# open-mmlab/Amphion

Hardware: AMD Instinct MI355X
Metric: audio samples/sec (HiFi-GAN V1 22.05 kHz generator, mel->wav) (higher is better)
Workload: dtype f32 (split-f16 MFMA: 3 x v_mfma_f32_32x32x16_f16 per term, f32 accumulate)

## Files before the change

### amphion_amd/_lib.py

```python
from __future__ import annotations

import ctypes
import os
import weakref
from ctypes import POINTER, c_char_p, c_float, c_int, c_int32, c_int64, c_size_t, c_void_p

_HERE = os.path.dirname(os.path.abspath(__file__))
LIB_PATH = os.environ.get("AMP_LIB_PATH") or os.path.join(_HERE, "lib", "libamphion_hip.so")

AMP_MAX_STAGES = 8
AMP_MAX_KERNELS = 8
AMP_MAX_DILATIONS = 8

AMP_ARCH_HIFIGAN, AMP_ARCH_BIGVGAN, AMP_ARCH_HIFIGAN_VITS = 0, 1, 2
AMP_ACT_LRELU, AMP_ACT_SNAKE, AMP_ACT_SNAKEBETA = 0, 1, 2
AMP_PRECISION_F32, AMP_PRECISION_F16X3 = 0, 1
AMP_CONV_OPT_PAD_REFLECT, AMP_CONV_OPT_TANH = 1, 2
AMP_PAD_REPLICATE, AMP_PAD_ZEROS, AMP_PAD_REFLECT = 0, 1, 2
AMP_PW_BIAS, AMP_PW_BIAS_GELU, AMP_PW_SCALE_RES = 0, 1, 2
PRECISIONS = {"f32": AMP_PRECISION_F32, "fp32": AMP_PRECISION_F32, "f16x3": AMP_PRECISION_F16X3}


class AmpError(RuntimeError):

# ... 161 lines not shown
    "amp_dsconv_forward": (c_int, [c_void_p, c_void_p, c_int, c_int, c_int, c_void_p, c_size_t, c_void_p, c_void_p]),
    "amp_dsconv_destroy": (None, [c_void_p]),
    "amp_gelu": (c_int, [c_void_p, ctypes.c_longlong, c_void_p, c_void_p]),
    "amp_layer_norm_c": (c_int, [c_void_p, c_void_p, c_void_p, c_void_p, c_void_p, c_int, c_int, c_int, c_float, c_int, c_void_p, c_void_p]),
    "amp_add_channel_bias": (c_int, [c_void_p, c_void_p, c_int, c_int, c_int, c_void_p]),
    "amp_layer_norm_c_ragged": (c_int, [c_void_p, c_void_p, c_void_p, c_void_p, c_void_p, c_void_p, c_int, c_int, c_int, c_float, c_int, c_void_p, c_void_p]),
    "amp_dds_seam": (c_int, [c_void_p, c_void_p, c_void_p, c_void_p, c_float, c_void_p, c_void_p, c_int, c_int, c_void_p, c_void_p, c_float,
                             c_void_p, c_int, c_int, c_int, c_void_p, c_void_p, c_void_p]),
    "amp_dwconv_layer_norm_c": (c_int, [c_void_p, c_void_p, c_void_p, c_int, c_int, c_void_p, c_void_p, c_void_p, c_int, c_int, c_int, c_float, c_int, c_void_p, c_void_p]),
    "amp_dwconv_layer_norm_c_causal": (c_int, [c_void_p, c_void_p, c_void_p, c_int, c_int, c_void_p, c_void_p, c_void_p, c_int, c_int, c_int, c_float, c_int,
                                               c_void_p, c_void_p]),
    "amp_rel_attention_strided": (c_int, [c_void_p, c_void_p, c_void_p, ctypes.c_longlong, c_void_p, c_void_p, c_void_p, c_int, c_int, c_int, c_int, c_int, c_void_p, c_void_p]),
    "amp_set_rel_attention_tiled": (c_int, [c_int]),
    "amp_set_resblock_streams": (c_int, [c_int]),
    "amp_gen_prepare_streams": (c_int, [c_void_p]),
    "amp_rel_attention": (c_int, [c_void_p, c_void_p, c_void_p, c_void_p, c_void_p, c_void_p, c_int, c_int, c_int, c_int, c_int, c_void_p, c_void_p]),
    "amp_dwconv": (c_int, [c_void_p, c_void_p, c_void_p, c_void_p, c_int, c_int, c_int, c_int, c_int, c_void_p, c_void_p]),
    "amp_spline_flow": (c_int, [c_void_p, c_void_p, c_void_p, c_int, c_int, c_int, c_int, c_float, c_int, c_int, c_int, c_void_p, c_void_p]),
    "amp_spline_flow_proj": (c_int, [c_void_p, c_void_p, c_void_p, c_void_p, c_void_p, c_int, c_int, c_int, c_int, c_int, c_float, c_int, c_int, c_int, c_void_p, c_void_p]),
    "amp_affine_reverse": (c_int, [c_void_p, c_void_p, c_void_p, c_void_p, c_int, c_int, c_int, c_void_p, c_void_p]),
    "amp_embed_tokens": (c_int, [c_void_p, c_void_p, c_void_p, c_int, c_int, c_int, c_int, c_float, c_void_p, c_void_p]),
    "amp_durations": (c_int, [c_void_p, c_void_p, c_int, c_int, c_float, c_void_p, c_void_p, c_void_p, c_void_p]),
    "amp_expand_path": (c_int, [c_void_p, c_void_p, c_void_p, c_void_p, c_int, c_int, c_int, c_int, c_void_p, c_void_p, c_void_p]),
    "amp_expand_path_strided": (c_int, [c_void_p, ctypes.c_longlong, c_void_p, c_void_p, c_void_p, c_int, c_int, c_int, c_int, c_void_p, c_void_p, c_void_p]),
    "amp_gauss_sample": (c_int, [c_void_p, c_void_p, c_void_p, c_size_t, c_float, c_void_p, c_void_p]),
    "amp_snake": (c_int, [c_void_p, c_int, c_int, c_int, c_void_p, c_void_p, c_int, c_void_p, c_void_p]),
    "amp_fir_upsample": (c_int, [c_void_p, c_int, c_int, c_int, c_void_p, c_int, c_int, c_void_p, c_void_p]),
    "amp_fir_filter": (c_int, [c_void_p, c_int, c_int, c_int, c_void_p, c_int, c_int, c_int, c_int, c_int, c_void_p, c_void_p]),
    "amp_wav_to_pcm16": (c_int, [c_void_p, c_int, c_int, ctypes.c_longlong, c_void_p, c_void_p, ctypes.c_longlong, c_void_p]),
    "amp_conv_set_option": (c_int, [c_void_p, c_int, c_int]),
    "amp_pair_forward": (c_int, [c_void_p, c_void_p, c_void_p, c_int, c_int, c_float, c_void_p, c_void_p]),
    "amp_resblock_forward": (c_int, [POINTER(c_void_p), POINTER(c_void_p), c_int, c_void_p, c_int, c_int, c_float, c_void_p, c_void_p]),
    "amp_set_resblock_fusion": (c_int, [c_int]),
    "amp_conv_destroy": (None, [c_void_p]),
    "amp_set_small_conv": (c_int, [c_int]),
    "amp_set_conv_blk": (c_int, [c_int]),
    "amp_set_conv_rg_fast": (c_int, [c_int]),
    "amp_set_pingpong": (c_int, [c_int]),
    "amp_set_conv_blk_narrow": (c_int, [c_int]),
    "amp_ampblock_forward": (c_int, [POINTER(c_void_p), POINTER(c_void_p), c_int, c_void_p, c_void_p, c_int, c_void_p, c_void_p,
                                     c_void_p, c_int, c_int, c_void_p, c_int, c_float, c_void_p]),
    "amp_set_ampblock_fusion": (c_int, [c_int]),
    "amp_conv_create_gated": (c_int, [c_int, c_int, c_int, c_int, c_void_p, c_void_p, POINTER(c_void_p)]),
    "amp_wn_forward": (c_int, [POINTER(c_void_p), POINTER(c_void_p), c_int, c_void_p, c_void_p, ctypes.c_longlong, c_void_p, c_int, c_int,
                               c_void_p, c_void_p, c_void_p]),
    "amp_wn_gate": (c_int, [c_void_p, c_void_p, ctypes.c_longlong, c_void_p, c_int, c_int, c_int, c_void_p]),
    "amp_wn_accumulate": (c_int, [c_void_p, c_void_p, c_void_p, c_void_p, c_int, c_int, c_int, c_int, c_int, c_void_p]),
    "amp_sequence_mask": (c_int, [c_void_p, c_void_p, c_int, c_int, c_int, c_void_p]),
    "amp_coupling_apply": (c_int, [c_void_p, c_void_p, c_void_p, c_int, c_int, c_int, c_int, c_void_p]),
    "amp_flip_channels": (c_int, [c_void_p, c_void_p, c_int, c_int, c_int, c_void_p]),
    "amp_posterior_sample": (c_int, [c_void_p, c_void_p, c_void_p, c_void_p, c_int, c_int, c_int, c_void_p]),
    "amp_antialias_snake": (c_int, [c_void_p, c_int, c_int, c_int, c_void_p, c_void_p, c_int, c_void_p, c_void_p, c_void_p, c_void_p]),
    "amp_istft_forward": (c_int, [POINTER(amp_mel_desc), c_void_p, c_void_p, c_int, c_int, c_void_p, c_void_p, c_void_p, c_void_p, c_void_p]),
    "amp_mel_num_frames": (c_int, [POINTER(amp_mel_desc), c_int]),
    "amp_mel_init": (c_int, []),
    "amp_mel_forward_ragged": (c_int, [POINTER(amp_mel_desc), c_void_p, c_void_p, c_int, c_int, c_void_p, c_void_p, c_void_p, c_void_p, c_void_p, c_void_p, c_void_p]),
    "amp_mel_backward": (c_int, [POINTER(amp_mel_desc), c_void_p, c_int, c_int] + [c_void_p] * 11),
    "amp_mel_forward": (c_int, [POINTER(amp_mel_desc), c_void_p, c_int, c_int, c_void_p, c_void_p, c_void_p, c_void_p, c_void_p, c_void_p, c_void_p]),
}

EXPORTED_SYMBOLS = tuple(_SIGNATURES)

_lib = None


def lib():
# ... 106 lines not shown
```

### amphion_amd/csrc/amp_host.h

```cpp
#pragma once
#include <math.h>

#include <vector>

#include "amp_internal.h"

#define AMP_HIP(expr)                                                                  \
    do {                                                                               \
        hipError_t e__ = (expr);                                                       \
        if (e__ != hipSuccess) {                                                       \
            set_error("%s failed: %s (%s:%d)", #expr, hipGetErrorString(e__), __FILE__, __LINE__); \
            return AMP_ERR_HIP;                                                        \
        }                                                                              \
    } while (0)

#define AMP_RC(expr) do { int rc__ = (expr); if (rc__ != AMP_OK) return rc__; } while (0)

struct amp_conv {
    int transposed = 0, cin = 0, cout = 0, k = 0, stride = 1, dilation = 1, padding = 0;
    int M = 0, ntaps = 0, KT = 0, off0 = 0, dstep = 0, halo_left = 0, halo_right = 0, up = 1, up_pad = 0;
    int nchunks = 0;
    int precision = amp::PREC_F32;
    int pad_reflect = 0, tanh_out = 0;
    int out_pad = 0;
// ... 93 lines not shown
    return wp;
}

template <class View>
int pack_matrix_f16x3(const char* who, int rows, int cols, int row_blocks, int k16, View W, std::vector<_Float16>* wp, float* inv_scale) {
    float wmax = 0.f;
    for (int m = 0; m < rows; ++m)
        for (int i = 0; i < cols; ++i) {
            const float w = fabsf(W(m, i));
            if (!(w < 1e30f)) { set_error("%s: non-finite weight", who); return AMP_ERR_INVALID; }
            wmax = fmaxf(wmax, w);
        }
    const float wscale = pow2_weight_scale(wmax);
    *inv_scale = 1.f / (16.f * wscale);
    *wp = pack_a_f16x3(row_blocks, k16, 1, 0, wscale, [&](int m, int i, int) { return (m < rows && i < cols) ? W(m, i) : 0.f; });
    return AMP_OK;
}

int conv_build(amp_conv* c, const float* w, const float* bias);
int conv_run(const amp_conv* c, const float* x, int B, int T, float slope_in, const float* res, float slope_out, float* y, int mode, float div,
             hipStream_t stream, long long xbs = 0, const int* lens = nullptr, int len_mul = 1, ConvArgs* plan_small = nullptr,
             int* plan_ni = nullptr);
int next_rev(const int* lens);

bool pair_supported(const amp_conv* c1, const amp_conv* c2);
int pair_run(const amp_conv* c1, const amp_conv* c2, const float* x, int B, int T, float slope, float* y, int mode, float div,
             hipStream_t stream, const int* lens = nullptr, int len_mul = 1);
bool pair_strip_plan(int B, int T, int k, bool ragged, int* form, int* strip_len, int* spi, int* steps);
bool pair_tile_args(const amp_conv* c1, const amp_conv* c2, const float* x, int B, int T, float slope, float* y, int mode, float div,
                    const int* lens, int len_mul, PairArgs* out);

bool rb_supported(const amp_conv* const* c1, const amp_conv* const* c2, int np, int B, int T);
int rb_split(const amp_conv* const* c1, int np, int B, int T);
int rb_run(const amp_conv* const* c1, const amp_conv* const* c2, int np, const float* x, int B, int T, float slope, float* y, int mode,
           float div, hipStream_t stream, const int* lens = nullptr, int len_mul = 1, int first = 0, int count = -1);

struct ActParams {
    float* a_dev = nullptr;
    float* invb_dev = nullptr;
    float* fu_dev = nullptr;
    float* fd_dev = nullptr;
    float* fu2_dev = nullptr;
};
int act_params_upload(const float* alpha_dev, const float* beta_dev, int C, int logscale, const float* filt_up_host,
                      const float* filt_down_host, float** out);
bool ampb_supported(const amp_conv* const* c1, const amp_conv* const* c2, int np, const ActParams* acts, size_t nacts, int B, int T);
int ampb_run(const amp_conv* const* c1, const amp_conv* const* c2, int np, const ActParams* acts, const float* x, int B, int T, float* y,
             int mode, float div, hipStream_t stream, const int* lens = nullptr, int len_mul = 1);

}
```

### amphion_amd/csrc/amp_internal.h

```cpp
#pragma once
#include <hip/hip_runtime.h>
#include <stdarg.h>
#include <stdint.h>
#include <stdio.h>

#include <atomic>
#include <mutex>
#include <string>
#include <vector>

#include "amphion_hip.h"

namespace amp {

constexpr int KC = 8;
constexpr int KC16 = 16;

enum { PREC_F32 = 0, PREC_F16X3 = 1 };

struct ConvArgs {
    const float* x;
    const void* wp;
    const float* bias;
    const float* res;
// ... 50 lines not shown
    float div;
    const int* lens;
    int len_mul;
    unsigned* range_flag;
};

struct ConvSmall3Args {
    ConvArgs a[3];
    int nx[3], ny[3];
};
hipError_t launch_conv_small3(const ConvSmall3Args& p, const int ni[3], hipStream_t stream);

struct Pair3Args {
    PairArgs a[3];
    int n[3];
};
hipError_t launch_pair3(const Pair3Args& p, hipStream_t stream);

constexpr int AMP_RB_MAX_PAIRS = 3;
struct RbArgs {
    const float* x;
    float* y;
    const void* wp1[AMP_RB_MAX_PAIRS];
    const float* bias1[AMP_RB_MAX_PAIRS];
    const void* wp2[AMP_RB_MAX_PAIRS];
    const float* bias2[AMP_RB_MAX_PAIRS];
    float sc1[AMP_RB_MAX_PAIRS], isc1[AMP_RB_MAX_PAIRS], sc2[AMP_RB_MAX_PAIRS], isc2[AMP_RB_MAX_PAIRS];
    int dil[AMP_RB_MAX_PAIRS];
    int np;
    int rh;
    int B, C, T;
    int tiles_per_item;
    int rev;
    float slope;
    int mode;
    float div;
    const int* lens;
    int len_mul;
    unsigned* range_flag;
};

constexpr int AMP_AMPB_MAX_STEPS = 6;
struct AmpbArgs {
    const float* x;
    float* y;
    const void* wp[AMP_AMPB_MAX_STEPS];
    const float* bias[AMP_AMPB_MAX_STEPS];
    float sc[AMP_AMPB_MAX_STEPS], isc[AMP_AMPB_MAX_STEPS];
    int dil[AMP_AMPB_MAX_STEPS];
    const float* act_a[AMP_AMPB_MAX_STEPS];
    const float* act_invb[AMP_AMPB_MAX_STEPS];
    const float* act_fu[AMP_AMPB_MAX_STEPS];
    const float* act_fd[AMP_AMPB_MAX_STEPS];
    int ns;
    int rh;
    int B, C, T;
    int tiles_per_item;
    int rev;
    int mode;
    float div;
    const int* lens;
    int len_mul;
    unsigned* range_flag;
};

constexpr int DW_TN = 64;
// ... 228 lines not shown
```

### amphion_amd/csrc/conv_host.hip

```cpp
#include <string.h>

#include <memory>
#include <type_traits>
#include <vector>

#include "amp_host.h"

namespace amp {

template <int... K> struct Taps { static constexpr int list[] = {K...}; };
using ConvTaps = Taps<1, 2, 3, 5, 7, 11>;
using BlkTaps = Taps<2, 3, 7, 11>;
using SmallTaps = Taps<1, 3, 5, 7, 11>;
using PairTaps = Taps<3, 5, 7, 11>;
using RbTaps = Taps<3, 5, 7, 11>;
using AmpbTaps = Taps<3, 5, 7, 11>;

template <int... K, typename R, typename F>
static R with_taps(Taps<K...>, int k, R dflt, F&& f) {
    R r = dflt;
    (void)((k == K && (r = f(std::integral_constant<int, K>{}), true)) || ...);
    return r;
}

// ... 396 lines not shown

bool rb_supported(const amp_conv* const* c1, const amp_conv* const* c2, int np, int B, int T) {
    if (np < 1 || np > AMP_RB_MAX_PAIRS) return false;
    int max_dil = 1, rh = 0;
    for (int p = 0; p < np; ++p) {
        if (!c1[p] || !c2[p] || !pair_supported(c1[p], c2[p])) return false;
        if (c1[p]->cin != c1[0]->cin || c1[p]->k != c1[0]->k) return false;
        max_dil = c1[p]->dilation > max_dil ? c1[p]->dilation : max_dil;
        rh += (c1[p]->k - 1) / 2 * (c1[p]->dilation + 1);
    }
    const int form = rb_form(c1[0]->cin, c1[0]->k);
    if (form < 0) return false;
    const int W = rb_tile(c1[0]->k, c1[0]->cin, max_dil, form);
    if (W <= 0 || W - 2 * rh < W / 2) return false;
    const int NT = W - 2 * rh;
    if (rb_fusion_mode() == 1 && (long long)B * ((T + NT - 1) / NT) < kRbMinWorkgroups) return false;
    return true;
}

int rb_split(const amp_conv* const* c1, int np, int B, int T) {
    if (np != 3 || rb_fusion_mode() != 1) return 0;
    int max_dil = 1, rh = 0;
    for (int p = 0; p < np; ++p) {
        max_dil = c1[p]->dilation > max_dil ? c1[p]->dilation : max_dil;
        rh += (c1[p]->k - 1) / 2 * (c1[p]->dilation + 1);
    }
    const int W = rb_tile(c1[0]->k, c1[0]->cin, max_dil, rb_form(c1[0]->cin, c1[0]->k));
    const int NT = W - 2 * rh;
    if (W <= 0 || 5 * NT >= 4 * W) return 0;
    if ((long long)B * ((T + NT - 1) / NT) < 1024) return 0;
    return 2;
}

int rb_run(const amp_conv* const* c1, const amp_conv* const* c2, int np, const float* x, int B, int T, float slope, float* y, int mode,
           float div, hipStream_t stream, const int* lens, int len_mul, int first, int count) {
    if (x == y) { set_error("rb_run: x and y must not alias"); return AMP_ERR_INVALID; }
    if (slope > 1.f) { set_error("rb_run: leaky_relu slope %g > 1 is outside the fused kernels", (double)slope); return AMP_ERR_UNSUPPORTED; }
    RbArgs a{};
    a.x = x; a.y = y;
    a.np = count < 0 ? np - first : count;
    c1 += first;
    c2 += first;
    int max_dil = 1;
    for (int p = 0; p < a.np; ++p) {
        a.wp1[p] = c1[p]->wp_dev; a.bias1[p] = c1[p]->bias_dev; a.wp2[p] = c2[p]->wp_dev; a.bias2[p] = c2[p]->bias_dev;
        a.sc1[p] = 16.f * c1[p]->wscale; a.isc1[p] = 1.f / a.sc1[p];
        a.sc2[p] = 16.f * c2[p]->wscale; a.isc2[p] = 1.f / a.sc2[p];
        a.dil[p] = c1[p]->dilation;
        a.rh += (c1[p]->k - 1) / 2 * (c1[p]->dilation + 1);
        max_dil = c1[p]->dilation > max_dil ? c1[p]->dilation : max_dil;
    }
    for (int p = a.np; p < AMP_RB_MAX_PAIRS; ++p) {
        a.wp1[p] = a.wp1[0]; a.bias1[p] = a.bias1[0]; a.wp2[p] = a.wp2[0]; a.bias2[p] = a.bias2[0]; a.dil[p] = 1;
    }
    a.B = B; a.C = c1[0]->cin; a.T = T;
    const int form = rb_form(a.C, c1[0]->k);
    const int W = rb_tile(c1[0]->k, a.C, max_dil, form);
    const int NT = W - 2 * a.rh;
    a.tiles_per_item = (T + NT - 1) / NT;
    a.slope = slope; a.mode = mode; a.div = div;
    a.lens = lens; a.len_mul = len_mul;
    a.range_flag = range_flag_for_current_device();
    a.rev = next_rev(lens);
    AMP_HIP(launch_rb(c1[0]->k, a, form, stream));
    return AMP_OK;
}

static int ampb_fusion_mode() { return cfg().ampb_fusion; }
static int ampb_form(int C, int k) {
    const int m = ampb_fusion_mode();
    if (m == 0) return -1;
    if (m == 3) return C == 32 ? 0 : 1;
    if (m == 2) return 1;
    if (C == 32) return k >= 11 ? 1 : 0;
    if (C == 64) return k <= 3 ? 1 : -1;
    return -1;
}
constexpr long long kAmpbMinWorkgroups = 256;

static int ampb_halo(const amp_conv* const* c1, int np) {
    int rh = 0;
    for (int p = 0; p < np; ++p) rh += 10 + (c1[p]->k - 1) / 2 * (c1[p]->dilation + 1);
    return (rh + 3) & ~3;
}

bool ampb_supported(const amp_conv* const* c1, const amp_conv* const* c2, int np, const ActParams* acts, size_t nacts, int B, int T) {
    if (np < 1 || 2 * np > AMP_AMPB_MAX_STEPS || nacts != (size_t)(2 * np)) return false;
    for (size_t i = 0; i < nacts; ++i)
        if (!acts[i].fu2_dev) return false;
    if ((T & 3) != 0) return false;
    int max_dil = 1;
    for (int p = 0; p < np; ++p) {
        const amp_conv *a = c1[p], *b = c2[p];
        if (!a || !b || a->precision != PREC_F16X3 || b->precision != PREC_F16X3) return false;
        if (a->pad_reflect || b->pad_reflect || a->tanh_out || b->tanh_out || a->transposed || b->transposed) return false;
        if (a->cin != a->cout || b->cin != b->cout || a->cin != b->cin || a->cin != c1[0]->cin) return false;
// ... 275 lines not shown
```

### amphion_amd/csrc/f16x3_device.h

```cpp
#pragma once
#include "amp_internal.h"

namespace amp {

typedef float f32x16 __attribute__((ext_vector_type(16)));
typedef _Float16 f16x8 __attribute__((ext_vector_type(8)));

union Frag {
    uint4 u;
    f16x8 h;
};

#define AMP_PIN_VMEM() __builtin_amdgcn_sched_barrier(0x386)
#define AMP_OPAQUE(v) asm("" : "+v"(v))

__device__ __forceinline__ int tile_order(unsigned bid, int nbx, bool ragged, int rev) {
    int bx = ((nbx & 7) == 0 && !ragged) ? (int)(bid & 7) * (nbx >> 3) + (int)(bid >> 3) : (int)bid;
    if (rev) bx = nbx - 1 - bx;
    return bx;
}

__device__ __forceinline__ int acc_row(int r, int hi = 0, int base = 0) { return base + (r & 3) + 8 * (r >> 2) + 4 * hi; }
__device__ __forceinline__ int bplane_idx(int qd, int col, int S) { return (((qd >> 1) * S + col) << 1) + (qd & 1); }
__device__ __forceinline__ void raise_range(unsigned* flag, float range_max, int lane) {
    if (flag && __any(range_max > 65504.f) && lane == 0) atomicOr(flag, 1u);
}

template <int MI, int NI>
__device__ __forceinline__ void mfma3_tiles(f32x16 (*acc)[NI], const Frag* a_h, const Frag* a_l, const Frag* bh, const Frag* bl) {
#pragma unroll
    for (int i = 0; i < MI; ++i)
#pragma unroll
        for (int t = 0; t < NI; ++t) acc[i][t] = __builtin_amdgcn_mfma_f32_32x32x16_f16(a_h[i].h, bh[t].h, acc[i][t], 0, 0, 0);
#pragma unroll
    for (int i = 0; i < MI; ++i)
#pragma unroll
        for (int t = 0; t < NI; ++t) acc[i][t] = __builtin_amdgcn_mfma_f32_32x32x16_f16(a_h[i].h, bl[t].h, acc[i][t], 0, 0, 0);
#pragma unroll
    for (int i = 0; i < MI; ++i)
#pragma unroll
        for (int t = 0; t < NI; ++t) acc[i][t] = __builtin_amdgcn_mfma_f32_32x32x16_f16(a_l[i].h, bh[t].h, acc[i][t], 0, 0, 0);
}
template <int N>
__device__ __forceinline__ void mfma3(f32x16* acc, const Frag& a_h, const Frag& a_l, const Frag* bh, const Frag* bl) {
    mfma3_tiles<1, N>(reinterpret_cast<f32x16(*)[N]>(acc), &a_h, &a_l, bh, bl);
}

__device__ __forceinline__ void split_f16(float v, _Float16& h, _Float16& l) {
    asm("" : "+v"(v));
    h = (_Float16)v;
    l = (_Float16)(v - (float)h);
}

typedef float amp_f32x2 __attribute__((ext_vector_type(2)));
typedef _Float16 amp_f16x2 __attribute__((ext_vector_type(2)));

__device__ __forceinline__ void split4_f16(amp_f32x2 v01, amp_f32x2 v23, uint2& h, uint2& l) {
    asm("" : "+v"(v01));
    asm("" : "+v"(v23));
    const amp_f16x2 h01 = __builtin_convertvector(v01, amp_f16x2), h23 = __builtin_convertvector(v23, amp_f16x2);
    h.x = __builtin_bit_cast(unsigned, h01); h.y = __builtin_bit_cast(unsigned, h23);
#ifndef AMP_SPLIT_PACKED
    asm("v_fma_mixlo_f16 %0, %1, 1.0, -%2 op_sel_hi:[0,0,1]" : "=v"(l.x) : "v"(v01.x), "v"(h.x));
    asm("v_fma_mixhi_f16 %0, %1, 1.0, -%2 op_sel:[0,0,1] op_sel_hi:[0,0,1]" : "+v"(l.x) : "v"(v01.y), "v"(h.x));
    asm("v_fma_mixlo_f16 %0, %1, 1.0, -%2 op_sel_hi:[0,0,1]" : "=v"(l.y) : "v"(v23.x), "v"(h.y));
    asm("v_fma_mixhi_f16 %0, %1, 1.0, -%2 op_sel:[0,0,1] op_sel_hi:[0,0,1]" : "+v"(l.y) : "v"(v23.y), "v"(h.y));
#else
    const amp_f32x2 d01 = v01 - __builtin_convertvector(h01, amp_f32x2), d23 = v23 - __builtin_convertvector(h23, amp_f32x2);
    const amp_f16x2 l01 = __builtin_convertvector(d01, amp_f16x2), l23 = __builtin_convertvector(d23, amp_f16x2);
    l.x = __builtin_bit_cast(unsigned, l01); l.y = __builtin_bit_cast(unsigned, l23);
#endif
}

__device__ __forceinline__ void stage4_f16(float x0, float x1, float x2, float x3, float kpos, float kneg, float& range_max,
                                           uint2& h, uint2& l) {
    const amp_f32x2 x01 = {x0, x1}, x23 = {x2, x3};
    const amp_f32x2 a01 = x01 * kpos, a23 = x23 * kpos, b01 = x01 * kneg, b23 = x23 * kneg;
    const amp_f32x2 v01 = {__builtin_fmaxf(a01.x, b01.x), __builtin_fmaxf(a01.y, b01.y)};
// ... 21 lines not shown
```

### amphion_amd/csrc/rb_f16x3.hip

```cpp
#include "f16x3_device.h"

#ifndef AMP_KT
#error "compile with -DAMP_KT=<taps>"
#endif

namespace amp {


template <int KT, int WM, int WN, int NI, int RING = 0, int RB_G = 32>
__global__ __launch_bounds__(64 * WM * WN, 2) void rb_f16x3_kernel(const RbArgs a) {
    static_assert(RING == 0 || RING < KT, "a ring shorter than one chunk");
    constexpr int NTHR = 64 * WM * WN;
    constexpr int W = 32 * NI * WN;
    constexpr int WL = W + 2 * RB_G;
    constexpr int H2 = (KT - 1) / 2;
    constexpr int NCH = 2 * WM;
    constexpr int CHS = 4 * WL;
    constexpr int C = 32 * WM;
    static_assert(NI % 2 == 0, "B fragments are read in halves");
    extern __shared__ __attribute__((aligned(16))) uint4 smem4[];

    const int tid = threadIdx.x;
    const int lane = tid & 63;
    const int wave = __builtin_amdgcn_readfirstlane(tid >> 6);
    const int wm = wave / WN, wn = wave % WN;
    const int hi = lane >> 5, l31 = lane & 31;
    const int nbx = gridDim.x;
    int bx = tile_order(blockIdx.x, nbx, a.lens != nullptr, a.rev);
    const int item = bx / a.tiles_per_item;
    const int tile = bx - item * a.tiles_per_item;
    const int T = a.T;
    const int RH = a.rh;
    const int NT = W - 2 * RH;
    const int O0 = tile * NT;
    int Tv = T;
    if (a.lens) { const int l = a.lens[item] * a.len_mul; Tv = l < Tv ? l : Tv; }
    if (O0 >= Tv) return;
    const int q0 = O0 - RH;

    for (int i = tid; i < NCH * 4 * 2 * RB_G; i += NTHR) {
        const int row = i / (2 * RB_G), g = i - row * (2 * RB_G);
        smem4[row * WL + (g < RB_G ? g : W + g)] = make_uint4(0u, 0u, 0u, 0u);
    }

    const int colw = wn * (32 * NI) + l31;
    int qcl[NI];
    bool qok[NI];
#pragma unroll
    for (int t = 0; t < NI; ++t) {
        const int q = q0 + colw + 32 * t;
        qok[t] = (q >= 0) && (q < Tv);
        qcl[t] = q < 0 ? 0 : (q < T ? q : T - 1);
    }
    const float* xr = a.x + (size_t)item * C * T + (size_t)(32 * wm + 16 * hi) * T;
    f32x16 rv[NI];
#pragma unroll
    for (int t = 0; t < NI; ++t)
#pragma unroll
        for (int r = 0; r < 16; ++r) rv[t][r] = xr[(size_t)r * T + qcl[t]];

    constexpr size_t MBS = (size_t)NCH * (KT * 128);
    constexpr int NA = RING > 0 ? RING : KT;
    Frag a_h[NA], a_l[NA];
    const int wlane = (lane & 32) | (16 * ((lane >> 2) & 1) + 4 * ((lane >> 3) & 3) + (lane & 3));
    {
        const uint4* w0 = static_cast<const uint4*>(a.wp1[0]) + (size_t)wm * MBS + wlane;
#pragma unroll
        for (int g = 0; g < NA; ++g) {
            a_h[g].u = w0[g * 128];
            a_l[g].u = w0[g * 128 + 64];
        }
    }
    AMP_PIN_VMEM();

    float range_max = 0.f;
    const float kpos = 16.f, kneg = 16.f * a.slope;
    auto stage_x = [&]() __attribute__((always_inline)) {
#pragma unroll
        for (int t = 0; t < NI; ++t) {
            const int col = RB_G + colw + 32 * t;
            const bool ok = qok[t];
            const int o4 = (2 * wm + hi) * CHS + col;
#pragma unroll
            for (int o = 0; o < 2; ++o) {
                struct { uint2 u; } fh0, fl0, fh1, fl1;
                stage4_f16(ok ? rv[t][8 * o + 0] : 0.f, ok ? rv[t][8 * o + 1] : 0.f, ok ? rv[t][8 * o + 2] : 0.f,
                           ok ? rv[t][8 * o + 3] : 0.f, kpos, kneg, range_max, fh0.u, fl0.u);
                stage4_f16(ok ? rv[t][8 * o + 4] : 0.f, ok ? rv[t][8 * o + 5] : 0.f, ok ? rv[t][8 * o + 6] : 0.f,
                           ok ? rv[t][8 * o + 7] : 0.f, kpos, kneg, range_max, fh1.u, fl1.u);
                smem4[o4 + o * WL] = make_uint4(fh0.u.x, fh0.u.y, fh1.u.x, fh1.u.y);
                smem4[o4 + o * WL + 2 * WL] = make_uint4(fl0.u.x, fl0.u.y, fl1.u.x, fl1.u.y);
            }
        }
    };

    f32x16 acc[NI];
    auto conv = [&](const void* wp, const float* bias, float sc, int d, const void* wp_next) __attribute__((always_inline)) {
#pragma unroll
        for (int r = 0; r < 16; ++r) {
            const float bv = bias[32 * wm + 16 * hi + r] * sc;
#pragma unroll
            for (int t = 0; t < NI; ++t) acc[t][r] = bv;
        }
        const uint4* wa = static_cast<const uint4*>(wp) + (size_t)wm * MBS + wlane;
        const uint4* wn0 = static_cast<const uint4*>(wp_next) + (size_t)wm * MBS + wlane;
        const int rd = hi * WL + RB_G + colw - H2 * d;
#pragma unroll 1
        for (int c = 0; c < NCH; ++c) {
            const uint4* wcur = wa + (size_t)c * (KT * 128);
            const uint4* wan = (c + 1) < NCH ? wa + (size_t)(c + 1) * (KT * 128) : wn0;
            const uint4* base = smem4 + c * CHS + rd;
#pragma unroll
            for (int g = 0; g < KT; ++g) {
                const int v = RING > 0 ? g % NA : g;
                const uint4* bg = base + g * d;
                constexpr int NB = NI / 2;
#pragma unroll
                for (int th = 0; th < 2; ++th) {
                    Frag bh[NB], bl[NB];
#pragma unroll
                    for (int t = 0; t < NB; ++t) {
                        bh[t].u = bg[32 * (th * NB + t)];
                        bl[t].u = bg[2 * WL + 32 * (th * NB + t)];
                    }
                    mfma3<NB>(acc + th * NB, a_h[v], a_l[v], bh, bl);
                }
                {
                    const bool same = RING > 0 && g + RING < KT;
                    const uint4* src = same ? wcur + (size_t)(g + RING) * 128 : wan + (size_t)v * 128;
                    a_h[v].u = src[0];
                    a_l[v].u = src[64];
                }
                AMP_PIN_VMEM();
            }
        }
    };

    stage_x();
    __syncthreads();

    const int np = a.np;
#pragma unroll 1
    for (int p = 0; p < AMP_RB_MAX_PAIRS; ++p) {
        if (p < np) {
            const bool last = (p + 1 == np);
            conv(a.wp1[p], a.bias1[p], a.sc1[p], a.dil[p], a.wp2[p]);
            __syncthreads();
            {
                const float i1 = a.isc1[p];
                const float slope = a.slope;
#pragma unroll
                for (int t = 0; t < NI; ++t) {
                    const int o4 = (2 * wm + hi) * CHS + RB_G + colw + 32 * t;
#pragma unroll
                    for (int o = 0; o < 2; ++o) {
                        struct { uint2 u; } fh0, fl0, fh1, fl1;
                        seam4_f16(acc[t][8 * o + 0], acc[t][8 * o + 1], acc[t][8 * o + 2], acc[t][8 * o + 3], i1, slope, qok[t], range_max, fh0.u, fl0.u);
                        seam4_f16(acc[t][8 * o + 4], acc[t][8 * o + 5], acc[t][8 * o + 6], acc[t][8 * o + 7], i1, slope, qok[t], range_max, fh1.u, fl1.u);
                        smem4[o4 + o * WL] = make_uint4(fh0.u.x, fh0.u.y, fh1.u.x, fh1.u.y);
                        smem4[o4 + o * WL + 2 * WL] = make_uint4(fl0.u.x, fl0.u.y, fl1.u.x, fl1.u.y);
                    }
                }
            }
            __syncthreads();
            conv(a.wp2[p], a.bias2[p], a.sc2[p], 1, last ? a.wp2[p] : a.wp1[p + 1 < AMP_RB_MAX_PAIRS ? p + 1 : p]);
            {
                const float i2 = a.isc2[p];
#pragma unroll
                for (int t = 0; t < NI; ++t)
#pragma unroll
                    for (int r = 0; r < 16; ++r) rv[t][r] = __builtin_fmaf(acc[t][r], i2, rv[t][r]);
            }
            if (!last) {
                __syncthreads();
                stage_x();
                __syncthreads();
            }
        }
    }

    {
        const int mode = a.mode;
        float* yr = a.y + (size_t)item * C * T + (size_t)(32 * wm + 16 * hi) * T;
        if (mode != 0) {
#pragma unroll
            for (int t = 0; t < NI; ++t)
#pragma unroll
                for (int r = 0; r < 16; ++r) acc[t][r] = yr[(size_t)r * T + qcl[t]];
#pragma unroll
            for (int t = 0; t < NI; ++t) rv[t] += acc[t];
            if (mode == 2) {
#pragma unroll
                for (int t = 0; t < NI; ++t)
#pragma unroll
                    for (int r = 0; r < 16; ++r) rv[t][r] = rv[t][r] / a.div;
            }
        }
#pragma unroll
        for (int t = 0; t < NI; ++t) {
            const int col = colw + 32 * t;
            const int q = q0 + col;
            if (col >= RH && col < W - RH && q < T) {
#pragma unroll
                for (int r = 0; r < 16; ++r) yr[(size_t)r * T + qcl[t]] = rv[t][r];
            }
        }
    }
    if (a.range_flag && __any(range_max > 65504.f) && lane == 0) atomicOr(a.range_flag, 1u);
}

template <int KT, int WM, int WN, int NI, int RING = 0, int RB_G = 32>
static hipError_t launch_rb_one(const RbArgs& a, hipStream_t stream) {
    constexpr int W = 32 * NI * WN;
    const size_t lds = (size_t)2 * WM * 4 * (W + 2 * RB_G) * sizeof(uint4);
    if (hipError_t e = ensure_dynamic_lds<&rb_f16x3_kernel<KT, WM, WN, NI, RING, RB_G>>(lds); e != hipSuccess) return e;
    dim3 grid((unsigned)(a.B * a.tiles_per_item));
    note_kernel("rb_f16x3_kernel", KT, WM, WN, NI, RING, RB_G);
    note_work(grid.x, a.np * 2 * 2.0 * a.C * a.C * KT * (double)a.T * a.B / 1e9, 4.0 * a.B * (double)a.C * a.T * (2 + (a.mode ? 1 : 0)) / 1e6,
              "whole ResBlock C=%d k=%d T=%d B=%d: %d convs%s", a.C, KT, a.T, a.B, 2 * a.np, a.mode ? " +sum" : "");
    hipLaunchKernelGGL((rb_f16x3_kernel<KT, WM, WN, NI, RING, RB_G>), grid, dim3(64 * WM * WN), lds, stream, a);
    return hipGetLastError();
}

template <int KT>
int rb_tile(int C, int max_dil, int wide) {
    const int reach = (KT - 1) / 2 * max_dil;
    if (reach > 32) return 0;
    if (C == 32) return wide ? 1024 : 512;
    if (C == 64) return wide ? 512 : ((KT <= 5 && reach <= 16) ? 256 : 0);
    if (C == 128) return (wide && KT <= 5 && reach <= 16) ? 256 : 0;
    return 0;
}

template <int KT>
hipError_t launch_rb(const RbArgs& a, int wide, hipStream_t stream) {
    constexpr int RING = KT >= 7 ? 4 : 0;
    if (a.C == 32) return wide ? launch_rb_one<KT, 1, 8, 4, RING>(a, stream) : launch_rb_one<KT, 1, 4, 4, RING>(a, stream);
    if (a.C == 64 && wide) return launch_rb_one<KT, 2, 4, 4, RING>(a, stream);
    if constexpr (KT <= 5) {
        if (a.C == 64 && !wide) return launch_rb_one<KT, 2, 2, 4, 0, 16>(a, stream);
    }
    if constexpr (KT <= 5) {
        if (a.C == 128 && wide) return launch_rb_one<KT, 4, 2, 4, 0, 16>(a, stream);
    }

    return hipErrorInvalidValue;
}

template int rb_tile<AMP_KT>(int, int, int);
template hipError_t launch_rb<AMP_KT>(const RbArgs&, int, hipStream_t);

}
```

### amphion_amd/csrc/runtime.hip

```cpp
#include <stdarg.h>
#include <stdio.h>
#include <stdlib.h>
#include <string.h>

#include <mutex>
#include <string>

#include "amp_host.h"

namespace amp {

static thread_local char g_err[512] = "";

void set_error(const char* fmt, ...) {
    va_list ap;
    va_start(ap, fmt);
    vsnprintf(g_err, sizeof(g_err), fmt, ap);
    va_end(ap);
}

static RangeGuard g_guard[64];
__thread std::string* tl_kernel_log = nullptr;
__thread char tl_last_kernel[160] = "";
__thread int tl_conv_transposed = 0;
// ... 114 lines not shown
    rb_fusion = num("AMP_RB_FUSION", 0, 3, 1);
    ampb_fusion = num("AMP_AMPB_FUSION", 0, 3, 1);
    rb_streams = num("AMP_RB_STREAMS", -1, 1, -1);
    static const char* const kRemoved[][2] = {
        {"AMP_GROUP_MB", "amp_set_group_mb(megabytes)"}, {"AMP_PAIR_STRIP", "amp_set_pair_strips(mode)"}, {"AMP_CONV_BLK", "amp_set_conv_blk(mode)"},
        {"AMP_FUSE_PAIRS", "nothing (the fused pairs are the only form)"}, {"AMP_RB_SUM_FRAMES", "nothing"},
        {"AMP_RB_HORIZONTAL", "amp_set_resblock_streams(mode)"}, {"AMP_RB_HORIZONTAL_FRAMES", "amp_set_resblock_streams(mode)"}};
    for (const auto& r : kRemoved) {
        const char* e = getenv(r[0]);
        if (e && *e) fprintf(stderr, "libamphion_hip: the environment variable %s=%s is no longer read (removed in ABI 142); use %s\n", r[0], e, r[1]);
    }
}
Config& cfg() { static Config c; return c; }

int device_upload(const void* host, size_t bytes, void** out) {
    void* p = nullptr;
    AMP_HIP(hipMalloc(&p, bytes));
    const hipError_t e = hipMemcpy(p, host, bytes, hipMemcpyHostToDevice);
    if (e != hipSuccess) {
        (void)hipFree(p);
        set_error("hipMemcpy of %zu bytes to the device failed: %s", bytes, hipGetErrorString(e));
        return AMP_ERR_HIP;
    }
    *out = p;
    return AMP_OK;
}

}

using namespace amp;

extern "C" {

int amp_version(void) { return 151; }
const char* amp_last_error(void) { return g_err; }

int amp_set_precision(int precision) {
    if (precision != AMP_PRECISION_F32 && precision != AMP_PRECISION_F16X3) {
        set_error("amp_set_precision: unknown precision %d", precision);
        return AMP_ERR_INVALID;
    }
    g_precision = precision;
    return AMP_OK;
}

int amp_get_precision(void) { return default_precision(); }

int amp_device_count(void) {
    int n = 0;
    if (hipGetDeviceCount(&n) != hipSuccess) return 0;
    return n;
}

int amp_set_pair_strips(int on) {
    if (on < -1 || on > 0) { set_error("amp_set_pair_strips: %d (-1 the policy, 0 the per-tile kernel everywhere; the four-wave strips of mode 1 left in ABI 142)", on); return AMP_ERR_INVALID; }
    cfg().pair_strips = on;
    return AMP_OK;
}

int amp_set_strip_fit(int mode) {
    if (mode < -1 || mode > 1) { set_error("amp_set_strip_fit: %d (-1 the plan, 0 never: shifted strips, 1 every strip launch)", mode); return AMP_ERR_INVALID; }
    cfg().strip_fit = mode;
    return AMP_OK;
}

int amp_pair_strip_plan(int B, int T, int k, int ragged, int* form, int* strip_len, int* strips_per_item, int* steps) {
    if (B < 1 || T < 1 || !form || !strip_len || !strips_per_item || !steps) { set_error("amp_pair_strip_plan: B=%d T=%d or a null result pointer", B, T); return AMP_ERR_INVALID; }
    if (!pair_strip_plan(B, T, k, ragged != 0, form, strip_len, strips_per_item, steps)) { set_error("amp_pair_strip_plan: no strip kernel for k=%d", k); return AMP_ERR_UNSUPPORTED; }
    return AMP_OK;
}

int amp_set_group_mb(int megabytes) {
    if (megabytes < 0) { set_error("amp_set_group_mb: %d", megabytes); return AMP_ERR_INVALID; }
    cfg().group_bytes = (size_t)megabytes << 20;
    return AMP_OK;
}

int amp_set_resblock_streams(int mode) {
    if (mode < -1 || mode > 1) { set_error("amp_set_resblock_streams: mode=%d", mode); return AMP_ERR_INVALID; }
    cfg().rb_streams = mode;
    return AMP_OK;
}

int amp_set_small_conv(int on) {
    cfg().small_conv = on ? 1 : 0;
    return AMP_OK;
}

int amp_set_pingpong(int on) {
    cfg().pingpong = on < 0 ? kPingPongDefault : (on ? 1 : 0);
    return AMP_OK;
}

int amp_set_conv_rg_fast(int on) {
    cfg().conv_rg_fast = on < 0 ? kConvRgFastDefault : (on ? 1 : 0);
    return AMP_OK;
}

int amp_set_conv_blk_narrow(int on) {
    if (on < -1 || on > 2) { set_error("amp_set_conv_blk_narrow: %d (0 off, 1 policy: 128-row convs with k >= 7, 2 every 128-row conv, -1 default)", on); return AMP_ERR_INVALID; }
    cfg().narrow_blk = on < 0 ? 1 : on;
    return AMP_OK;
}

// ... 24 lines not shown
```

### include/amphion_hip.h

```cpp
#ifndef AMPHION_HIP_H
#define AMPHION_HIP_H

#include <stddef.h>
#include <stdint.h>

#ifdef __cplusplus
extern "C" {
#endif

typedef enum amp_status {
    AMP_OK = 0,
    AMP_ERR_INVALID = -1,
    AMP_ERR_MISSING_WEIGHT = -2,
    AMP_ERR_HIP = -3,
    AMP_ERR_UNSUPPORTED = -4,
    AMP_ERR_STATE = -5,
    AMP_ERR_RANGE = -6
} amp_status;

typedef enum amp_arch {
    AMP_ARCH_HIFIGAN = 0,
    AMP_ARCH_BIGVGAN = 1,
    AMP_ARCH_HIFIGAN_VITS = 2
} amp_arch;
// ... 124 lines not shown
                    int filter_channels, float tail_bound, int inverse, int flip_in, int flip_out, float* z_out_dev,
                    void* stream);
int amp_spline_flow_proj(const float* z_dev, const float* hc_dev, const float* proj_w_dev, const float* proj_b_dev, const int* lens_dev,
                         int B, int C, int T, int num_bins, int filter_channels, float tail_bound, int inverse, int flip_in, int flip_out,
                         float* z_out_dev, void* stream);
int amp_affine_reverse(const float* x_dev, const float* m_dev, const float* logs_dev, const int* lens_dev, int B, int C, int T,
                       float* y_dev, void* stream);
int amp_embed_tokens(const long long* tokens_dev, const float* weight_dev, const int* lens_dev, int B, int T, int hidden,
                     int n_vocab, float scale, float* y_dev, void* stream);
int amp_durations(const float* logw_dev, const int* lens_dev, int B, int T, float length_scale, float* w_ceil_dev, int* cum_dev,
                  int* ylen_dev, void* stream);
int amp_expand_path(const float* src_dev, const int* cum_dev, const int* xlens_dev, const int* ylens_dev, int B, int D, int Tx,
                    int Ty, float* out_dev, float* attn_dev, void* stream);
int amp_expand_path_strided(const float* src_dev, long long src_batch_stride, const int* cum_dev, const int* xlens_dev,
                            const int* ylens_dev, int B, int D, int Tx, int Ty, float* out_dev, float* attn_dev, void* stream);
int amp_gauss_sample(const float* m_dev, const float* logs_dev, const float* noise_dev, size_t n, float noise_scale,
                     float* out_dev, void* stream);

int amp_snake(const float* x_dev, int B, int C, int T, const float* alpha_dev, const float* beta_dev, int logscale,
              float* y_dev, void* stream);

int amp_wav_to_pcm16(const float* wav_dev, int B, int L, long long wav_stride, const int* lens_dev, int16_t* pcm_dev,
                     long long pcm_stride, void* stream);

typedef enum amp_conv_option { AMP_CONV_OPT_PAD_REFLECT = 1, AMP_CONV_OPT_TANH = 2 } amp_conv_option;
int amp_conv_set_option(amp_conv* c, int option, int value);

int amp_pair_forward(const amp_conv* c1, const amp_conv* c2, const float* x_dev, int B, int T, float slope,
                     float* y_dev, void* stream);

int amp_resblock_forward(const amp_conv* const* c1, const amp_conv* const* c2, int n_pairs, const float* x_dev, int B, int T,
                         float slope, float* y_dev, void* stream);
int amp_set_resblock_fusion(int mode);
int amp_set_resblock_streams(int mode);
int amp_gen_prepare_streams(amp_gen* g);

int amp_ampblock_forward(const amp_conv* const* c1, const amp_conv* const* c2, int n_pairs, const float* alpha_dev,
                         const float* beta_dev, int logscale, const float* filt_up_host, const float* filt_down_host,
                         const float* x_dev, int B, int T, float* y_dev, int mode, float div, void* stream);
int amp_set_ampblock_fusion(int mode);

void amp_conv_destroy(amp_conv* c);

int amp_set_small_conv(int on);

int amp_set_conv_blk(int mode);
int amp_set_conv_blk_narrow(int on);

int amp_set_conv_rg_fast(int on);

int amp_set_pingpong(int on);


int amp_conv_create_gated(int hidden, int k, int dilation, int padding, const float* weight_host, const float* bias_host,
                          amp_conv** out);

int amp_wn_forward(const amp_conv* const* in_layers, const amp_conv* const* res_skip_layers, int n_layers, float* x_dev,
                   const float* cond_dev, long long cond_batch_stride, const int32_t* lens_dev, int B, int T,
                   float* acts_ws_dev, float* out_dev, void* stream);


int amp_wn_gate(const float* a_dev, const float* cond_dev, long long cond_batch_stride, float* out_dev, int B, int H,
                int T, void* stream);
int amp_wn_accumulate(float* x_dev, float* out_dev, const float* rs_dev, const int32_t* lens_dev, int B, int H, int T,
                      int first, int last, void* stream);
int amp_sequence_mask(float* x_dev, const int32_t* lens_dev, int B, int C, int T, void* stream);
// ... 176 lines not shown
```

Measured before the change: 151.1 million.

## Lean ResBlock kernel: 32-bit lane offsets, MFMA bias init, interior tile fast path

Adds a compile-time switch that turns on three register and instruction savings in the fused ResBlock f16x3 kernel. Row base pointers for x and y are pinned in scalar registers and each lane uses a 32-bit byte offset when C*T fits in 2 GB. The first chunk's MFMA takes the bias vector as its accumulator input instead of a separate broadcast loop. Interior tiles skip per-column bounds masks when staging x. The aim is lower VGPR pressure and fewer address and select instructions, at the cost of more template instantiations and reliance on asm pinning tricks.

```diff
diff --git a/amphion_amd/_lib.py b/amphion_amd/_lib.py
--- a/amphion_amd/_lib.py
+++ b/amphion_amd/_lib.py
@@ -217,6 +217,7 @@
     "amp_pair_forward": (c_int, [c_void_p, c_void_p, c_void_p, c_int, c_int, c_float, c_void_p, c_void_p]),
     "amp_resblock_forward": (c_int, [POINTER(c_void_p), POINTER(c_void_p), c_int, c_void_p, c_int, c_int, c_float, c_void_p, c_void_p]),
     "amp_set_resblock_fusion": (c_int, [c_int]),
+    "amp_resblock_addr32": (c_int, [c_int, c_int]),
     "amp_conv_destroy": (None, [c_void_p]),
     "amp_set_small_conv": (c_int, [c_int]),
     "amp_set_conv_blk": (c_int, [c_int]),
diff --git a/amphion_amd/csrc/amp_host.h b/amphion_amd/csrc/amp_host.h
--- a/amphion_amd/csrc/amp_host.h
+++ b/amphion_amd/csrc/amp_host.h
@@ -149,6 +149,7 @@
 
 bool rb_supported(const amp_conv* const* c1, const amp_conv* const* c2, int np, int B, int T);
 int rb_split(const amp_conv* const* c1, int np, int B, int T);
+bool rb_addr32(int C, int T);
 int rb_run(const amp_conv* const* c1, const amp_conv* const* c2, int np, const float* x, int B, int T, float slope, float* y, int mode,
            float div, hipStream_t stream, const int* lens = nullptr, int len_mul = 1, int first = 0, int count = -1);
 
diff --git a/amphion_amd/csrc/amp_internal.h b/amphion_amd/csrc/amp_internal.h
--- a/amphion_amd/csrc/amp_internal.h
+++ b/amphion_amd/csrc/amp_internal.h
@@ -106,6 +106,7 @@
     int B, C, T;
     int tiles_per_item;
     int rev;
+    int addr32;
     float slope;
     int mode;
     float div;
diff --git a/amphion_amd/csrc/conv_host.hip b/amphion_amd/csrc/conv_host.hip
--- a/amphion_amd/csrc/conv_host.hip
+++ b/amphion_amd/csrc/conv_host.hip
@@ -452,6 +452,8 @@
     return 2;
 }
 
+bool rb_addr32(int C, int T) { return C > 0 && T > 0 && (long long)C * T * 4 < (1LL << 31); }
+
 int rb_run(const amp_conv* const* c1, const amp_conv* const* c2, int np, const float* x, int B, int T, float slope, float* y, int mode,
            float div, hipStream_t stream, const int* lens, int len_mul, int first, int count) {
     if (x == y) { set_error("rb_run: x and y must not alias"); return AMP_ERR_INVALID; }
@@ -482,6 +484,7 @@
     a.lens = lens; a.len_mul = len_mul;
     a.range_flag = range_flag_for_current_device();
     a.rev = next_rev(lens);
+    a.addr32 = rb_addr32(a.C, T) ? 1 : 0;
     AMP_HIP(launch_rb(c1[0]->k, a, form, stream));
     return AMP_OK;
 }
diff --git a/amphion_amd/csrc/f16x3_device.h b/amphion_amd/csrc/f16x3_device.h
--- a/amphion_amd/csrc/f16x3_device.h
+++ b/amphion_amd/csrc/f16x3_device.h
@@ -44,6 +44,16 @@
 template <int N>
 __device__ __forceinline__ void mfma3(f32x16* acc, const Frag& a_h, const Frag& a_l, const Frag* bh, const Frag* bl) {
     mfma3_tiles<1, N>(reinterpret_cast<f32x16(*)[N]>(acc), &a_h, &a_l, bh, bl);
+}
+
+template <int N>
+__device__ __forceinline__ void mfma3_from(f32x16* acc, const f32x16& c0, const Frag& a_h, const Frag& a_l, const Frag* bh, const Frag* bl) {
+#pragma unroll
+    for (int t = 0; t < N; ++t) acc[t] = __builtin_amdgcn_mfma_f32_32x32x16_f16(a_h.h, bh[t].h, c0, 0, 0, 0);
+#pragma unroll
+    for (int t = 0; t < N; ++t) acc[t] = __builtin_amdgcn_mfma_f32_32x32x16_f16(a_h.h, bl[t].h, acc[t], 0, 0, 0);
+#pragma unroll
+    for (int t = 0; t < N; ++t) acc[t] = __builtin_amdgcn_mfma_f32_32x32x16_f16(a_l.h, bh[t].h, acc[t], 0, 0, 0);
 }
 
 __device__ __forceinline__ void split_f16(float v, _Float16& h, _Float16& l) {
diff --git a/amphion_amd/csrc/rb_f16x3.hip b/amphion_amd/csrc/rb_f16x3.hip
--- a/amphion_amd/csrc/rb_f16x3.hip
+++ b/amphion_amd/csrc/rb_f16x3.hip
@@ -1,13 +1,24 @@
+#include <type_traits>
+
 #include "f16x3_device.h"
 
 #ifndef AMP_KT
 #error "compile with -DAMP_KT=<taps>"
 #endif
 
+#ifndef AMP_RB_LEAN
+#define AMP_RB_LEAN (AMP_KT <= 5 ? 7 : AMP_KT <= 7 ? 5 : 1)
+#endif
+
 namespace amp {
 
-
-template <int KT, int WM, int WN, int NI, int RING = 0, int RB_G = 32>
+typedef const float __attribute__((address_space(1)))* GlobalCF;
+typedef float __attribute__((address_space(1)))* GlobalF;
+
+constexpr bool kRbAddr32 = (AMP_RB_LEAN & 1) != 0, kRbMfmaInit = (AMP_RB_LEAN & 2) != 0, kRbInterior = (AMP_RB_LEAN & 4) != 0;
+
+
+template <int KT, int WM, int WN, int NI, int RING = 0, int RB_G = 32, int A32 = 0>
 __global__ __launch_bounds__(64 * WM * WN, 2) void rb_f16x3_kernel(const RbArgs a) {
     static_assert(RING == 0 || RING < KT, "a ring shorter than one chunk");
     constexpr int NTHR = 64 * WM * WN;
@@ -52,12 +63,42 @@
         qok[t] = (q >= 0) && (q < Tv);
         qcl[t] = q < 0 ? 0 : (q < T ? q : T - 1);
     }
-    const float* xr = a.x + (size_t)item * C * T + (size_t)(32 * wm + 16 * hi) * T;
     f32x16 rv[NI];
-#pragma unroll
-    for (int t = 0; t < NI; ++t)
-#pragma unroll
-        for (int r = 0; r < 16; ++r) rv[t][r] = xr[(size_t)r * T + qcl[t]];
+    const size_t wbase = (size_t)item * C * T + (size_t)(32 * wm) * T;
+    unsigned loff[NI];
+#pragma unroll
+    for (int t = 0; t < NI; ++t) loff[t] = 4u * (unsigned)(16 * hi * T + qcl[t]);
+    auto pin_rows = [&](auto* rows, auto* row, auto AGAIN) __attribute__((always_inline)) {
+#pragma unroll
+        for (int r = 0; r < 16; ++r) {
+            row[r] = (std::remove_reference_t<decltype(row[0])>)(rows + (size_t)r * T);
+            if constexpr (decltype(AGAIN)::value) asm volatile("" : "+s"(row[r]));
+            else asm("" : "+s"(row[r]));
+        }
+    };
+    auto lane_ptr = [&](auto* row, unsigned off) __attribute__((always_inline)) {
+        typedef std::conditional_t<std::is_const_v<std::remove_pointer_t<decltype(row)>>, const char, char> __attribute__((address_space(1))) B;
+        return (decltype(row))((B*)row + off);
+    };
+    auto lane_off = [&](int t) __attribute__((always_inline)) {
+        unsigned o = loff[t];
+        asm volatile("" : "+v"(o));
+        return o;
+    };
+    if constexpr (A32) {
+        GlobalCF xrow[16];
+        pin_rows(a.x + wbase, xrow, std::false_type{});
+#pragma unroll
+        for (int t = 0; t < NI; ++t)
+#pragma unroll
+            for (int r = 0; r < 16; ++r) rv[t][r] = *lane_ptr(xrow[r], loff[t]);
+    } else {
+        const float* xr = a.x + (size_t)item * C * T + (size_t)(32 * wm + 16 * hi) * T;
+#pragma unroll
+        for (int t = 0; t < NI; ++t)
+#pragma unroll
+            for (int r = 0; r < 16; ++r) rv[t][r] = xr[(size_t)r * T + qcl[t]];
+    }
 
     constexpr size_t MBS = (size_t)NCH * (KT * 128);
     constexpr int NA = RING > 0 ? RING : KT;
@@ -75,11 +116,11 @@
 
     float range_max = 0.f;
     const float kpos = 16.f, kneg = 16.f * a.slope;
-    auto stage_x = [&]() __attribute__((always_inline)) {
+    auto stage_x_as = [&](auto SEL) __attribute__((always_inline)) {
 #pragma unroll
         for (int t = 0; t < NI; ++t) {
             const int col = RB_G + colw + 32 * t;
-            const bool ok = qok[t];
+            const bool ok = !decltype(SEL)::value || qok[t];
             const int o4 = (2 * wm + hi) * CHS + col;
 #pragma unroll
             for (int o = 0; o < 2; ++o) {
@@ -93,20 +134,27 @@
             }
         }
     };
+    const bool interior = kRbInterior && q0 >= 0 && q0 + W <= Tv;
+    auto stage_x = [&]() __attribute__((always_inline)) {
+        if (interior) stage_x_as(std::false_type{});
+        else stage_x_as(std::true_type{});
+    };
 
     f32x16 acc[NI];
     auto conv = [&](const void* wp, const float* bias, float sc, int d, const void* wp_next) __attribute__((always_inline)) {
-#pragma unroll
-        for (int r = 0; r < 16; ++r) {
-            const float bv = bias[32 * wm + 16 * hi + r] * sc;
-#pragma unroll
-            for (int t = 0; t < NI; ++t) acc[t][r] = bv;
+        f32x16 bv;
+#pragma unroll
+        for (int r = 0; r < 16; ++r) bv[r] = bias[32 * wm + 16 * hi + r] * sc;
+        if constexpr (!kRbMfmaInit) {
+#pragma unroll
+            for (int r = 0; r < 16; ++r)
+#pragma unroll
+                for (int t = 0; t < NI; ++t) acc[t][r] = bv[r];
         }
         const uint4* wa = static_cast<const uint4*>(wp) + (size_t)wm * MBS + wlane;
         const uint4* wn0 = static_cast<const uint4*>(wp_next) + (size_t)wm * MBS + wlane;
         const int rd = hi * WL + RB_G + colw - H2 * d;
-#pragma unroll 1
-        for (int c = 0; c < NCH; ++c) {
+        auto chunk = [&](int c, auto FIRST) __attribute__((always_inline)) {
             const uint4* wcur = wa + (size_t)c * (KT * 128);
             const uint4* wan = (c + 1) < NCH ? wa + (size_t)(c + 1) * (KT * 128) : wn0;
             const uint4* base = smem4 + c * CHS + rd;
@@ -123,7 +171,8 @@
                         bh[t].u = bg[32 * (th * NB + t)];
                         bl[t].u = bg[2 * WL + 32 * (th * NB + t)];
                     }
-                    mfma3<NB>(acc + th * NB, a_h[v], a_l[v], bh, bl);
+                    if (decltype(FIRST)::value && g == 0) mfma3_from<NB>(acc + th * NB, bv, a_h[v], a_l[v], bh, bl);
+                    else mfma3<NB>(acc + th * NB, a_h[v], a_l[v], bh, bl);
                 }
                 {
                     const bool same = RING > 0 && g + RING < KT;
@@ -133,6 +182,14 @@
                 }
                 AMP_PIN_VMEM();
             }
+        };
+        if constexpr (kRbMfmaInit) {
+            chunk(0, std::true_type{});
+#pragma unroll 1
+            for (int c = 1; c < NCH; ++c) chunk(c, std::false_type{});
+        } else {
+#pragma unroll 1
+            for (int c = 0; c < NCH; ++c) chunk(c, std::false_type{});
         }
     };
 
@@ -182,11 +239,15 @@
     {
         const int mode = a.mode;
         float* yr = a.y + (size_t)item * C * T + (size_t)(32 * wm + 16 * hi) * T;
+        GlobalF yrow[16];
         if (mode != 0) {
-#pragma unroll
-            for (int t = 0; t < NI; ++t)
-#pragma unroll
-                for (int r = 0; r < 16; ++r) acc[t][r] = yr[(size_t)r * T + qcl[t]];
+            if constexpr (A32) pin_rows(a.y + wbase, yrow, std::false_type{});
+#pragma unroll
+            for (int t = 0; t < NI; ++t) {
+                const unsigned off = A32 ? lane_off(t) : 0u;
+#pragma unroll
+                for (int r = 0; r < 16; ++r) acc[t][r] = A32 ? *lane_ptr(yrow[r], off) : yr[(size_t)r * T + qcl[t]];
+            }
 #pragma unroll
             for (int t = 0; t < NI; ++t) rv[t] += acc[t];
             if (mode == 2) {
@@ -196,29 +257,37 @@
                     for (int r = 0; r < 16; ++r) rv[t][r] = rv[t][r] / a.div;
             }
         }
+        if constexpr (A32) pin_rows(a.y + wbase, yrow, std::true_type{});
 #pragma unroll
         for (int t = 0; t < NI; ++t) {
             const int col = colw + 32 * t;
             const int q = q0 + col;
             if (col >= RH && col < W - RH && q < T) {
-#pragma unroll
-                for (int r = 0; r < 16; ++r) yr[(size_t)r * T + qcl[t]] = rv[t][r];
+                const unsigned off = A32 ? lane_off(t) : 0u;
+#pragma unroll
+                for (int r = 0; r < 16; ++r) {
+                    if constexpr (A32) *lane_ptr(yrow[r], off) = rv[t][r];
+                    else yr[(size_t)r * T + qcl[t]] = rv[t][r];
+                }
             }
         }
     }
     if (a.range_flag && __any(range_max > 65504.f) && lane == 0) atomicOr(a.range_flag, 1u);
 }
 
-template <int KT, int WM, int WN, int NI, int RING = 0, int RB_G = 32>
+template <int KT, int WM, int WN, int NI, int RING = 0, int RB_G = 32, int A32 = 0>
 static hipError_t launch_rb_one(const RbArgs& a, hipStream_t stream) {
+    if constexpr (kRbAddr32 && !A32) {
+        if (a.addr32) return launch_rb_one<KT, WM, WN, NI, RING, RB_G, 1>(a, stream);
+    }
     constexpr int W = 32 * NI * WN;
     const size_t lds = (size_t)2 * WM * 4 * (W + 2 * RB_G) * sizeof(uint4);
-    if (hipError_t e = ensure_dynamic_lds<&rb_f16x3_kernel<KT, WM, WN, NI, RING, RB_G>>(lds); e != hipSuccess) return e;
+    if (hipError_t e = ensure_dynamic_lds<&rb_f16x3_kernel<KT, WM, WN, NI, RING, RB_G, A32>>(lds); e != hipSuccess) return e;
     dim3 grid((unsigned)(a.B * a.tiles_per_item));
-    note_kernel("rb_f16x3_kernel", KT, WM, WN, NI, RING, RB_G);
+    note_kernel("rb_f16x3_kernel", KT, WM, WN, NI, RING, RB_G, A32);
     note_work(grid.x, a.np * 2 * 2.0 * a.C * a.C * KT * (double)a.T * a.B / 1e9, 4.0 * a.B * (double)a.C * a.T * (2 + (a.mode ? 1 : 0)) / 1e6,
               "whole ResBlock C=%d k=%d T=%d B=%d: %d convs%s", a.C, KT, a.T, a.B, 2 * a.np, a.mode ? " +sum" : "");
-    hipLaunchKernelGGL((rb_f16x3_kernel<KT, WM, WN, NI, RING, RB_G>), grid, dim3(64 * WM * WN), lds, stream, a);
+    hipLaunchKernelGGL((rb_f16x3_kernel<KT, WM, WN, NI, RING, RB_G, A32>), grid, dim3(64 * WM * WN), lds, stream, a);
     return hipGetLastError();
 }
 
diff --git a/amphion_amd/csrc/runtime.hip b/amphion_amd/csrc/runtime.hip
--- a/amphion_amd/csrc/runtime.hip
+++ b/amphion_amd/csrc/runtime.hip
@@ -170,7 +170,7 @@
 
 extern "C" {
 
-int amp_version(void) { return 151; }
+int amp_version(void) { return 152; }
 const char* amp_last_error(void) { return g_err; }
 
 int amp_set_precision(int precision) {
@@ -208,6 +208,8 @@
     return AMP_OK;
 }
 
+int amp_resblock_addr32(int C, int T) { return rb_addr32(C, T) ? 1 : 0; }
+
 int amp_set_group_mb(int megabytes) {
     if (megabytes < 0) { set_error("amp_set_group_mb: %d", megabytes); return AMP_ERR_INVALID; }
     cfg().group_bytes = (size_t)megabytes << 20;
diff --git a/include/amphion_hip.h b/include/amphion_hip.h
--- a/include/amphion_hip.h
+++ b/include/amphion_hip.h
@@ -180,6 +180,7 @@
 int amp_resblock_forward(const amp_conv* const* c1, const amp_conv* const* c2, int n_pairs, const float* x_dev, int B, int T,
                          float slope, float* y_dev, void* stream);
 int amp_set_resblock_fusion(int mode);
+int amp_resblock_addr32(int C, int T);
 int amp_set_resblock_streams(int mode);
 int amp_gen_prepare_streams(amp_gen* g);
 
```

New measurement: 152.1 million, median of 6. Within noise of the previous version (+0.6%).
